# hal0zer0/openwurli

Measured on AMD Instinct MI355X. Metric: audio samples/s, 64-voice full chain (x real-time @48 kHz = value / 48000), higher is better.
Workload: dtype f64

## Files before the change

openwurli_amd/csrc/ow_chain_dev.h:

```cpp
#pragma once
#include "ow_voice_dev.h"

namespace owdev {

OW_DEV double fast_exp(double x0) {
    const double x = clampd(x0, -40.0, 40.0);
    const double SHIFT = 6755399441055744.0;
    const double z = x * 1.4426950408889634 + SHIFT;
    const long long n_i64 = __double_as_longlong(z) - __double_as_longlong(SHIFT);
    const double n = z - SHIFT;
    const double f = (x - n * 0.6931471803691238) - n * 1.9082149292705877e-10;
    const double p = 1.0 + f * (1.0 + f * (0.5 + f * (0.16666666666666607 + f * (0.04166666666665876 + f * 0.008333333333492337))));
    const double pow2n = __longlong_as_double((long long)(((unsigned long long)(1023 + n_i64)) << 52));
    return p * pow2n;
}

__device__ __noinline__ __attribute__((const)) double pnjlim_limited(double vnew, double vold, double vt, double vcrit) {
    if (vold >= 0.0) {
        const double arg = 1.0 + (vnew - vold) / vt;
        return arg > 0.0 ? vold + vt * log(arg) : vcrit;
    }
    return vt * log(vnew / vt);
}
OW_DEV double pnjlim(double vnew, double vold, double vt, double vcrit) {
// ... 383 lines not shown
}
OW_DEV double trem_shunt(double depth, double r_ldr) {
    const double r_upper = 50000.0 * (1.0 - depth);
    const double r_lower = 50000.0 * depth;
    const double top = r_upper > 0.0 ? ow_div(r_upper * 18000.0, r_upper + 18000.0) : 0.0;
    const double branch = 680.0 + r_ldr;
    const double low = r_lower > 0.0 ? ow_div(r_lower * branch, r_lower + branch) : 0.0;
    return top + low;
}

struct Smoother {
    double cur, target, step;
    uint32_t rem;
    OW_DEV double next() {
        if (rem > 0u) {
            cur += step;
            rem -= 1u;
            if (rem == 0u) cur = target;
        }
        return cur;
    }
    OW_DEV void retarget(double t, uint32_t ramp) {
        target = t;
        const double delta = t - cur;
        if (ramp == 0u) { cur = t; rem = 0u; return; }
        step = delta / (double)ramp;
        rem = ramp;
    }
};

OW_DEV double xor32(double x);
OW_DEV double xor32_t(double x) {
#ifdef OW_XOR32_SWAP
    return xor32(x);
#else
    return __shfl_xor(x, 32);
#endif
}
OW_DEV double xor32(double x) {
    const int lo = __double2loint(x), hi = __double2hiint(x);
    const auto a = __builtin_amdgcn_permlane32_swap(lo, lo, false, false);
    const auto b = __builtin_amdgcn_permlane32_swap(hi, hi, false, false);
    const bool low_half = (threadIdx.x & 63) < 32;
    return __hiloint2double(low_half ? b[1] : b[0], low_half ? a[1] : a[0]);
}

#define OW_P_IS 3.03e-14
#define OW_P_VT 0.026
struct DkSt { double j_cin, cin_prev, v[8], i_nl[2], v_nl[2], gm[2]; };
#ifdef OW_DBG_COUNTERS
extern __device__ unsigned long long g_ow_dbg[8];
#endif

OW_DEV double exp_bounded(double x) {
#ifdef OW_LIB_EXP
    return exp(x);
#else
    const double n = rint(x * __longlong_as_double(0x3ff71547652b82feLL));
    double r = __builtin_fma(__longlong_as_double((long long)0xbfe62e42fefa39efULL), n, x);
    r = __builtin_fma(__longlong_as_double((long long)0xbc7abc9e3b39803fULL), n, r);
    double p = __builtin_fma(__longlong_as_double(0x3e5ade156a5dcb37LL), r, __longlong_as_double(0x3e928af3fca7ab0cLL));
    p = __builtin_fma(r, p, __longlong_as_double(0x3ec71dee623fde64LL));
    p = __builtin_fma(r, p, __longlong_as_double(0x3efa01997c89e6b0LL));
    p = __builtin_fma(r, p, __longlong_as_double(0x3f2a01a014761f6eLL));
    p = __builtin_fma(r, p, __longlong_as_double(0x3f56c16c1852b7b0LL));
    p = __builtin_fma(r, p, __longlong_as_double(0x3f81111111122322LL));
    p = __builtin_fma(r, p, __longlong_as_double(0x3fa55555555502a1LL));
    p = __builtin_fma(r, p, __longlong_as_double(0x3fc5555555555511LL));
    p = __builtin_fma(r, p, __longlong_as_double(0x3fe000000000000bLL));
    p = __builtin_fma(r, p, 1.0);
    p = __builtin_fma(r, p, 1.0);
    return ldexp(p, (int)n);
#endif
}
OW_DEV double dk_clamp_vbe(double vbe) { return __builtin_fmin(__builtin_fmax(vbe, -1.0), 0.85); }
OW_DEV double dk_ic(double vbe) {
    return OW_P_IS * (exp_bounded(OW_DIV_C(dk_clamp_vbe(vbe), OW_P_VT)) - 1.0);
}
OW_DEV void dk_ic_gm(double vbe, double& ic, double& gm) {
    const double e = exp_bounded(OW_DIV_C(dk_clamp_vbe(vbe), OW_P_VT));
    ic = OW_P_IS * (e - 1.0);
    gm = (OW_P_IS / OW_P_VT) * e;
}
OW_DEV void dk_refresh_gm(DkSt& st) {
    double ic;
    dk_ic_gm(st.v_nl[0], ic, st.gm[0]);
    dk_ic_gm(st.v_nl[1], ic, st.gm[1]);
}

__device__ inline const OwConsts* k_reload(const OwConsts* K) {
    int z = 0;
    asm volatile("" : "+s"(z));
    return K + z;
}
__device__ inline double dk_step(DkSt& st, double input, double g_ldr, double g_ldr_prev, const OwConsts* __restrict__ K0) {
    const OwConsts* __restrict__ K = k_reload(K0);
    const double (*__restrict__ an)[8] = K->p_a_neg;
    const double* v = st.v;
    double rhs[8];
    rhs[0] = an[0][0] * v[0] + an[0][2] * v[2];
    rhs[1] = an[1][1] * v[1] + an[1][7] * v[7];
    rhs[2] = an[2][0] * v[0] + an[2][2] * v[2] + an[2][5] * v[5];
    rhs[3] = an[3][3] * v[3] + an[3][4] * v[4];
    rhs[4] = an[4][3] * v[3] + an[4][4] * v[4];
    rhs[5] = an[5][2] * v[2] + an[5][5] * v[5] + an[5][6] * v[6];
    rhs[6] = an[6][5] * v[5] + an[6][6] * v[6] + an[6][7] * v[7];
    rhs[7] = an[7][1] * v[1] + an[7][6] * v[6] + an[7][7] * v[7];
    rhs[7] -= g_ldr_prev * st.v[7];
    const double cin_now = K->p_g_cin * input + st.j_cin;
    rhs[0] += cin_now + st.cin_prev;
    rhs[1] += st.i_nl[0];
    rhs[2] -= st.i_nl[0];
    rhs[3] += st.i_nl[1];
    rhs[5] -= st.i_nl[1];
#pragma unroll
    for (int i = 0; i < 8; ++i) rhs[i] += K->p_two_w[i];
    double vpb[8];
    {
        const OwConsts* __restrict__ Kb = k_reload(K0);
#pragma unroll
        for (int i = 0; i < 4; ++i) {
            double sum = 0.0;
#pragma unroll
            for (int j = 0; j < 8; ++j) sum += Kb->p_s[i][j] * rhs[j];
            vpb[i] = sum;
// ... 20 lines not shown
    const double k11 = K->p_k[1][1] - sm_k * K->p_nv_sfb[1] * K->p_sfb_ni[1];
    double vn0 = st.v_nl[0], vn1 = st.v_nl[1];
    double ic0 = st.i_nl[0], ic1 = st.i_nl[1], gm0 = st.gm[0], gm1 = st.gm[1];
    bool done = false;
#ifdef OW_DBG_COUNTERS
    unsigned own_updates = 0u, wave_updates = 0u;
#endif
    for (int iter = 0; iter < 6; ++iter) {
        const double f0 = vn0 - p0 - k00 * ic0 - k01 * ic1;
        const double f1 = vn1 - p1 - k10 * ic0 - k11 * ic1;
        done = done || (fabs(f0) < 1e-9 && fabs(f1) < 1e-9);
        if (__builtin_amdgcn_ballot_w64(!done) == 0ull) break;
#ifdef OW_DBG_COUNTERS
        own_updates += done ? 0u : 1u; wave_updates += 1u;
#endif
        const double j00 = 1.0 - k00 * gm0, j01 = -k01 * gm1, j10 = -k10 * gm0, j11 = 1.0 - k11 * gm1;
        const double det = j00 * j11 - j01 * j10;
        done = done || fabs(det) < 1e-30;
        const double inv_det = ow_div(1.0, det);
        const double n0 = vn0 - inv_det * (j11 * f0 - j01 * f1);
        const double n1 = vn1 - inv_det * (j00 * f1 - j10 * f0);
        vn0 = done ? vn0 : n0;
        vn1 = done ? vn1 : n1;
        dk_ic_gm(vn0, ic0, gm0);
        dk_ic_gm(vn1, ic1, gm1);
    }
#ifdef OW_DBG_COUNTERS
    {
        const int ln = threadIdx.x & 63;
        atomicAdd(&g_ow_dbg[ln < 32 ? 0 : 1], (unsigned long long)own_updates);
        if (ln == 0) { atomicAdd(&g_ow_dbg[2], (unsigned long long)wave_updates); atomicAdd(&g_ow_dbg[3], 1ull); }
        unsigned m = own_updates;
        for (int o = 16; o > 0; o >>= 1) m = max(m, (unsigned)__shfl_xor((int)m, o));
        if (ln == 0) atomicAdd(&g_ow_dbg[4], (unsigned long long)m);
        if (ln == 32) atomicAdd(&g_ow_dbg[5], (unsigned long long)m);
    }
#endif
    K = k_reload(K0);
    const double dot = K->p_sfb_ni[0] * ic0 + K->p_sfb_ni[1] * ic1;
#pragma unroll
    for (int i = 0; i < 8; ++i) {
        const double s_ni_i = ic0 * K->p_sni_d1[i] + ic1 * K->p_sni_d2[i];
        st.v[i] = v_pred[i] + s_ni_i - sm_k * dot * K->p_s_fb_col[i];
    }
    st.cin_prev = cin_now;
    const double dv_cin = input - st.v[0];
    st.j_cin = -K->p_gc_1pc * dv_cin - K->p_c_cin * st.j_cin;
    st.i_nl[0] = ic0; st.i_nl[1] = ic1;
    st.v_nl[0] = vn0; st.v_nl[1] = vn1;
    st.gm[0] = gm0; st.gm[1] = gm1;
    return st.v[6];
}

OW_DEV void dk_rhs(const double (*__restrict__ an)[8], const DkSt& st, double input, double g_ldr_prev, double p_g_cin, double rhs[8], double& cin_now) {
    const double* v = st.v;
    rhs[0] = an[0][0] * v[0] + an[0][2] * v[2];
    rhs[1] = an[1][1] * v[1] + an[1][7] * v[7];
    rhs[2] = an[2][0] * v[0] + an[2][2] * v[2] + an[2][5] * v[5];
    rhs[3] = an[3][3] * v[3] + an[3][4] * v[4];
    rhs[4] = an[4][3] * v[3] + an[4][4] * v[4];
    rhs[5] = an[5][2] * v[2] + an[5][5] * v[5] + an[5][6] * v[6];
    rhs[6] = an[6][5] * v[5] + an[6][6] * v[6] + an[6][7] * v[7];
    rhs[7] = an[7][1] * v[1] + an[7][6] * v[6] + an[7][7] * v[7];
    rhs[7] -= g_ldr_prev * st.v[7];
    cin_now = p_g_cin * input + st.j_cin;
    rhs[0] += cin_now + st.cin_prev;
    rhs[1] += st.i_nl[0];
    rhs[2] -= st.i_nl[0];
    rhs[3] += st.i_nl[1];
    rhs[5] -= st.i_nl[1];
}
OW_DEV void dk_newton_update(double k00, double k01, double k10, double k11, double f0, double f1, bool& done,
                             double& vn0, double& vn1, double& ic0, double& ic1, double& gm0, double& gm1) {
    const double j00 = 1.0 - k00 * gm0, j01 = -k01 * gm1, j10 = -k10 * gm0, j11 = 1.0 - k11 * gm1;
    const double det = j00 * j11 - j01 * j10;
    done = done || fabs(det) < 1e-30;
    const double inv_det = ow_div(1.0, det);
    const double n0 = vn0 - inv_det * (j11 * f0 - j01 * f1);
    const double n1 = vn1 - inv_det * (j00 * f1 - j10 * f0);
    vn0 = done ? vn0 : n0;
    vn1 = done ? vn1 : n1;
    dk_ic_gm(vn0, ic0, gm0);
    dk_ic_gm(vn1, ic1, gm1);
}
OW_DEV double dk_close(const OwConsts* __restrict__ K, DkSt& st, const double v_pred[8], double sm_k, double cin_now, double input,
                       double vn0, double vn1, double ic0, double ic1, double gm0, double gm1) {
    const double dot = K->p_sfb_ni[0] * ic0 + K->p_sfb_ni[1] * ic1;
#pragma unroll
    for (int i = 0; i < 8; ++i) {
        const double s_ni_i = ic0 * K->p_sni_d1[i] + ic1 * K->p_sni_d2[i];
        st.v[i] = v_pred[i] + s_ni_i - sm_k * dot * K->p_s_fb_col[i];
    }
    st.cin_prev = cin_now;
    const double dv_cin = input - st.v[0];
    st.j_cin = -K->p_gc_1pc * dv_cin - K->p_c_cin * st.j_cin;
    st.i_nl[0] = ic0; st.i_nl[1] = ic1;
    st.v_nl[0] = vn0; st.v_nl[1] = vn1;
    st.gm[0] = gm0; st.gm[1] = gm1;
    return st.v[6];
}
__device__ inline void dk_step_pair(DkSt& sa, DkSt& sb, double in_a, double in_b, double g_ldr, double g_ldr_prev,
                                    const OwConsts* __restrict__ K0, double& out_a, double& out_b) {
    const OwConsts* __restrict__ K = k_reload(K0);
    double ra[8], rb[8], cin_a, cin_b;
    dk_rhs(K->p_a_neg, sa, in_a, g_ldr_prev, K->p_g_cin, ra, cin_a);
    dk_rhs(K->p_a_neg, sb, in_b, g_ldr_prev, K->p_g_cin, rb, cin_b);
#pragma unroll
    for (int i = 0; i < 8; ++i) { ra[i] += K->p_two_w[i]; rb[i] += K->p_two_w[i]; }
    double pa[8], pb[8];
    {
        const OwConsts* __restrict__ Kb = k_reload(K0);
#pragma unroll
        for (int i = 0; i < 4; ++i) {
            double sum_a = 0.0, sum_b = 0.0;
#pragma unroll
            for (int j = 0; j < 8; ++j) { const double s = Kb->p_s[i][j]; sum_a += s * ra[j]; sum_b += s * rb[j]; }
            pa[i] = sum_a; pb[i] = sum_b;
        }
        const OwConsts* __restrict__ Kc = k_reload(K0);
#pragma unroll
        for (int i = 4; i < 8; ++i) {
            double sum_a = 0.0, sum_b = 0.0;
#pragma unroll
            for (int j = 0; j < 8; ++j) { const double s = Kc->p_s[i][j]; sum_a += s * ra[j]; sum_b += s * rb[j]; }
            pa[i] = sum_a; pb[i] = sum_b;
        }
    }
    K = k_reload(K0);
    const double sm_k = ow_div(g_ldr, 1.0 + K->p_s_fb_fb * g_ldr);
    const double k00 = K->p_k[0][0] - sm_k * K->p_nv_sfb[0] * K->p_sfb_ni[0];
    const double k01 = K->p_k[0][1] - sm_k * K->p_nv_sfb[0] * K->p_sfb_ni[1];
    const double k10 = K->p_k[1][0] - sm_k * K->p_nv_sfb[1] * K->p_sfb_ni[0];
    const double k11 = K->p_k[1][1] - sm_k * K->p_nv_sfb[1] * K->p_sfb_ni[1];
    const double smv_a = sm_k * pa[7], smv_b = sm_k * pb[7];
#pragma unroll
    for (int i = 0; i < 8; ++i) { const double c = K->p_s_fb_col[i]; pa[i] = pa[i] - smv_a * c; pb[i] = pb[i] - smv_b * c; }
    const double p0a = pa[0] - pa[1], p1a = pa[2] - pa[3];
    const double p0b = pb[0] - pb[1], p1b = pb[2] - pb[3];
    double vn0a = sa.v_nl[0], vn1a = sa.v_nl[1], ic0a = sa.i_nl[0], ic1a = sa.i_nl[1], gm0a = sa.gm[0], gm1a = sa.gm[1];
    double vn0b = sb.v_nl[0], vn1b = sb.v_nl[1], ic0b = sb.i_nl[0], ic1b = sb.i_nl[1], gm0b = sb.gm[0], gm1b = sb.gm[1];
    bool done_a = false, done_b = false;
#pragma unroll
    for (int iter = 0; iter < 6; ++iter) {
        const double f0a = vn0a - p0a - k00 * ic0a - k01 * ic1a;
        const double f1a = vn1a - p1a - k10 * ic0a - k11 * ic1a;
        const double f0b = vn0b - p0b - k00 * ic0b - k01 * ic1b;
        const double f1b = vn1b - p1b - k10 * ic0b - k11 * ic1b;
        done_a = done_a || (fabs(f0a) < 1e-9 && fabs(f1a) < 1e-9);
        done_b = done_b || (fabs(f0b) < 1e-9 && fabs(f1b) < 1e-9);
        if (__builtin_amdgcn_ballot_w64(!(done_a && done_b)) == 0ull) break;
        dk_newton_update(k00, k01, k10, k11, f0a, f1a, done_a, vn0a, vn1a, ic0a, ic1a, gm0a, gm1a);
        dk_newton_update(k00, k01, k10, k11, f0b, f1b, done_b, vn0b, vn1b, ic0b, ic1b, gm0b, gm1b);
    }
    K = k_reload(K0);
    out_a = dk_close(K, sa, pa, sm_k, cin_a, in_a, vn0a, vn1a, ic0a, ic1a, gm0a, gm1a);
    out_b = dk_close(K, sb, pb, sm_k, cin_b, in_b, vn0b, vn1b, ic0b, ic1b, gm0b, gm1b);
}

__device__ __noinline__ void dk_dc_state(const OwConsts* __restrict__ K, double r_ldr, DkSt* out) {
    double w[8][16];
    for (int i = 0; i < 8; ++i)
        for (int j = 0; j < 8; ++j) { w[i][j] = K->p_g_dc_base[i][j]; w[i][8 + j] = (i == j) ? 1.0 : 0.0; }
    w[7][7] += 1.0 / r_ldr;
    for (int col = 0; col < 8; ++col) {
        int piv = col;
        double best = fabs(w[col][col]);
        for (int r = col + 1; r < 8; ++r)
            if (fabs(w[r][col]) > best) { best = fabs(w[r][col]); piv = r; }
        if (piv != col)
            for (int j = 0; j < 16; ++j) { const double t = w[col][j]; w[col][j] = w[piv][j]; w[piv][j] = t; }
        const double d = w[col][col];
        for (int j = 0; j < 16; ++j) w[col][j] /= d;
        for (int r = 0; r < 8; ++r) {
            if (r == col) continue;
            const double f = w[r][col];
            for (int j = 0; j < 16; ++j) w[r][j] -= f * w[col][j];
        }
    }
#define SDC(i, j) w[i][8 + (j)]
    const double kd00 = SDC(0, 1) - SDC(0, 2) - SDC(1, 1) + SDC(1, 2);
    const double kd01 = SDC(0, 3) - SDC(0, 5) - SDC(1, 3) + SDC(1, 5);
    const double kd10 = SDC(2, 1) - SDC(2, 2) - SDC(3, 1) + SDC(3, 2);
    const double kd11 = SDC(2, 3) - SDC(2, 5) - SDC(3, 3) + SDC(3, 5);
    double wv[8], sv[8];
    for (int i = 0; i < 8; ++i) wv[i] = K->p_two_w[i] * 0.5;
    for (int i = 0; i < 8; ++i) {
        double sum = 0.0;
        for (int j = 0; j < 8; ++j) sum += SDC(i, j) * wv[j];
        sv[i] = sum;
    }
    const double pd0 = sv[0] - sv[1], pd1 = sv[2] - sv[3];
    double vn0 = 0.56, vn1 = 0.66;
    for (int iter = 0; iter < 100; ++iter) {
        double ic0, gm0, ic1, gm1;
        dk_ic_gm(vn0, ic0, gm0);
        dk_ic_gm(vn1, ic1, gm1);
        const double f0 = vn0 - pd0 - kd00 * ic0 - kd01 * ic1;
        const double f1 = vn1 - pd1 - kd10 * ic0 - kd11 * ic1;
        if (fabs(f0) < 1e-12 && fabs(f1) < 1e-12) break;
        const double j00 = 1.0 - kd00 * gm0, j01 = -kd01 * gm1, j10 = -kd10 * gm0, j11 = 1.0 - kd11 * gm1;
        const double det = j00 * j11 - j01 * j10;
        const double inv_det = 1.0 / det;
        const double dv0 = inv_det * (j11 * f0 - j01 * f1);
        const double dv1 = inv_det * (j00 * f1 - j10 * f0);
        const double ms = 2.0 * OW_P_VT;
        vn0 -= clampd(dv0, -ms, ms);
        vn1 -= clampd(dv1, -ms, ms);
    }
    const double ic0 = dk_ic(vn0), ic1 = dk_ic(vn1);
    double rhs[8];
    for (int i = 0; i < 8; ++i) rhs[i] = wv[i];
    rhs[1] += ic0; rhs[2] -= ic0; rhs[3] += ic1; rhs[5] -= ic1;
    for (int i = 0; i < 8; ++i) {
        double sum = 0.0;
        for (int j = 0; j < 8; ++j) sum += SDC(i, j) * rhs[j];
        out->v[i] = sum;
    }
#undef SDC
    out->j_cin = K->p_g_cin * out->v[0];
    out->cin_prev = K->p_g_cin * out->v[0];
    out->i_nl[0] = dk_ic(vn0); out->i_nl[1] = dk_ic(vn1);
    out->v_nl[0] = vn0; out->v_nl[1] = vn1;
}
__device__ inline void dk_dc_reset(const OwConsts* __restrict__ K, double r_ldr, DkSt& st) {
    DkSt tmp;
    dk_dc_state(K, r_ldr, &tmp);
    st = tmp;
    dk_refresh_gm(st);
}

OW_DEV double allpass3(const double c0, const double c1, const double c2, double st[3], double x) {
    double y = c0 * x + st[0];
    st[0] = x - c0 * y;
    double y2 = c1 * y + st[1];
    st[1] = y - c1 * y2;
    double y3 = c2 * y2 + st[2];
    st[2] = y2 - c2 * y3;
    return y3;
}
#define OW_OS_A0 0.036681502163648
#define OW_OS_A1 0.248030921580110
#define OW_OS_A2 0.643184620136480
#define OW_OS_B0 0.110377634768680
#define OW_OS_B1 0.420399304190880
#define OW_OS_B2 0.854640112701920


__device__ inline double power_amp(double input) {
    const double A = 19000.0, H = 22.0, TOL = 1e-6;
    const double beta = 220.0 / (220.0 + 15000.0);
    const double clg = A / (1.0 + A * beta);
    double y = clampd(input * clg, -H + TOL, H - TOL);
#ifndef OW_DK_DIVERGENT_NEWTON
    bool done = false;
#endif
    for (int it = 0; it < 8; ++it) {
        const double error = input - beta * y;
        const double v = A * error;
        const double v_sq = v * v;
        const double vt_sq = 0.013 * 0.013;
        const double exp_term = exp(OW_DIV_C(-v_sq, 0.013 * 0.013));
        const double q = 0.1;
        const double cross_gain = q + (1.0 - q) * (1.0 - exp_term);
        const double v_cross = v * cross_gain;
        const double dcross_dv = cross_gain + v * (1.0 - q) * OW_DIV_C(2.0 * v, 0.013 * 0.013) * exp_term;
        const double tanh_val = tanh_fast(OW_DIV_C(v_cross, 22.0));
        const double f_val = H * tanh_val;
        const double f_deriv = (1.0 - tanh_val * tanh_val) * dcross_dv;
        const double residual = y - f_val;
        const double jac = 1.0 + A * beta * f_deriv;
        const double delta = ow_div(residual, jac);
#ifndef OW_DK_DIVERGENT_NEWTON
        y = done ? y : y - delta;
        done = done || fabs(delta) < TOL;
        if (__builtin_amdgcn_ballot_w64(!done) == 0ull) break;
#else
        y -= delta;
        if (fabs(delta) < TOL) break;
#endif
    }
    return OW_DIV_C(y, 22.0);
}

struct Bq { double b0, b1, b2, a1, a2, s1, s2; };
OW_DEV double bq_process(Bq& f, double x) {
    const double y = f.b0 * x + f.s1;
    f.s1 = f.b1 * x - f.a1 * y + f.s2;
    f.s2 = f.b2 * x - f.a2 * y;
    return y;
}
__device__ inline void bq_design(Bq& f, bool highpass, double fc, double q, double sr) {
    const double w0 = 2.0 * 3.14159265358979323846 * fc / sr;
    const double cw = cos(w0), sw = sin(w0);
    const double alpha = sw / (2.0 * q);
    const double a0 = 1.0 + alpha;
    if (highpass) { f.b0 = ((1.0 + cw) / 2.0) / a0; f.b1 = (-(1.0 + cw)) / a0; f.b2 = ((1.0 + cw) / 2.0) / a0; }
    else          { f.b0 = ((1.0 - cw) / 2.0) / a0; f.b1 = (1.0 - cw) / a0;    f.b2 = ((1.0 - cw) / 2.0) / a0; }
    f.a1 = (-2.0 * cw) / a0;
    f.a2 = (1.0 - alpha) / a0;
}
struct SpeakerSt {
    Bq hpf, lpf;
    double character, a2, a3, tc, ts;
};
__device__ inline void speaker_update(SpeakerSt& s, double sr) {
    const double c = s.character;
    bq_design(s.hpf, true, 20.0 * pow(30.0 / 20.0, c), 0.75, sr);
    bq_design(s.lpf, false, 20000.0 * pow(5500.0 / 20000.0, c), 0.707, sr);
    s.a2 = 0.2 * c;
    s.a3 = 0.6 * c;
    s.tc = 2.0 * c;
}
OW_DEV void speaker_set_character(SpeakerSt& s, double ch, double sr) {
    const double c = clampd(ch, 0.0, 1.0);
// ... 23 lines not shown
```

openwurli_amd/csrc/ow_dk_step_debug.h:

```cpp
#pragma once
#include "ow_chain_row.h"

namespace owdev {

enum { DKF_LANE = 0, DKF_PAIR = 1, DKF_WIDE = 2, DKF_ROW = 3 };

template <int FORM>
__global__ __launch_bounds__(64) void k_debug_dk_step(const OwConsts* __restrict__ K, const double* __restrict__ cs_in, const double* __restrict__ input,
                                                      const double* __restrict__ g_ldr, const double* __restrict__ g_ldr_prev, int n,
                                                      double* __restrict__ cs_out, double* __restrict__ out) {
    const int lane = threadIdx.x;
    const long long t = (long long)blockIdx.x * 64 + lane;
    if constexpr (FORM == DKF_LANE) {
        const bool valid = t < n;
        const int c = valid ? (int)t : n - 1;
        DkSt st;
        dk_load(st, cs_in, n, c, 0);
        const double o = dk_step(st, input[c], g_ldr[c], g_ldr_prev[c], K);
        if (valid) { dk_store(st, cs_out, n, c, 0); out[c] = o; }
    } else if constexpr (FORM == DKF_PAIR) {
        const long long ca = 2 * t, cb = 2 * t + 1;
        const bool va = ca < n, vb = cb < n;
        const int a = va ? (int)ca : n - 1, b = vb ? (int)cb : n - 1;
        DkSt sm, ss;
        dk_load(sm, cs_in, n, a, 0);
        dk_load(ss, cs_in, n, b, 0);
        double om, os;
        dk_step_pair(sm, ss, input[a], input[b], g_ldr[a], g_ldr_prev[a], K, om, os);
        if (va) { dk_store(sm, cs_out, n, a, 0); out[a] = om; }
        if (vb) { dk_store(ss, cs_out, n, b, 0); out[b] = os; }
    } else if constexpr (FORM == DKF_WIDE) {
        const int q = lane & 3;
        const long long cw = t >> 2;
        const bool valid = cw < n;
        const int c = valid ? (int)cw : n - 1;
        DkWideRows R;
        dk_wide_rows_load(R, K, q);
        DkSt st;
        dk_load(st, cs_in, n, c, 0);
        const double o = dk_step_wide(st, R, q, input[c], g_ldr[c], g_ldr_prev[c], K);
        if (valid && q == (c & 3)) { dk_store(st, cs_out, n, c, 0); out[c] = o; }
    } else {
        const long long cr = t >> 4;
        const bool valid = cr < n;
        const int c = valid ? (int)cr : n - 1;
        DkRowK R;
        dk_row_consts(R, K, lane);
        DkSt st;
        dk_load(st, cs_in, n, c, 0);
        const double o = dk_step_row(st, R, lane, input[c], g_ldr[c], g_ldr_prev[c]);
        if (valid && (lane & 15) == (c & 15)) { dk_store(st, cs_out, n, c, 0); out[c] = o; }
    }
}

}
```

openwurli_amd/csrc/ow_kernels.h:

```cpp
#pragma once
#include "ow_vm.h"
#include "ow_chain_dev.h"

namespace owdev {

#define OW_DATA_DECL __device__ const
#define OW_GEN_DATA_REINCLUDE
#include "../../data/ow_gen_data.h"
#undef OW_GEN_DATA_REINCLUDE
#undef OW_DATA_DECL

struct OwEngineOut {
    uint64_t silent_mask;
    uint64_t bad_main;
    uint64_t bad_steal;
    uint32_t sum_nonfinite;
    uint32_t out_nonfinite;
    uint32_t transient;
    uint32_t pad;
};

__device__ inline void mlp_raw_scalar(double in0, double in1, double raw[11]) {
    double h1[16], h2[16];
    for (int i = 0; i < 16; ++i) {
// ... 1055 lines not shown
            }
        }
        __syncthreads();
    }
    if (valid) {
        dk_store(st, cs, I, e, role ? CS_P_SHADOW : CS_P_MAIN);
        if (role == 0) {
            for (int i = 0; i < 3; ++i) { CSF(CS_OS_UA + i) = ua[i]; CSF(CS_OS_UB + i) = ub[i]; }
            CSF(CS_P_RLDR) = r_ldr; CSF(CS_P_GLDR) = g_ldr; CSF(CS_P_GPREV) = g_prev;
            smoother_store(sd, cs, I, e, CS_SM_DEPTH);
            const uint64_t fl = dbits(CSF(CS_FLAGS));
            if (fl & 1ull) CSF(CS_FLAGS) = bitsd(fl & ~1ull);
            if (nan_resets) {
                const uint64_t d = dbits(CSF(CS_DIAG));
                CSF(CS_DIAG) = bitsd((d & 0xFFFFFFFFull) | ((uint64_t)((uint32_t)(d >> 32) + nan_resets) << 32));
            }
        }
    }
}

#define OW_PPCHUNK 32
__global__ __launch_bounds__(64) __attribute__((amdgpu_waves_per_eu(2, 2)))
void k_preamp_pair(const OwConsts* __restrict__ K, double* __restrict__ cs, const OwEngineArgs* __restrict__ args,
                   const OwEngineOut* __restrict__ eout, const double* __restrict__ sum, const OwTremSrc tsrc,
                   double* __restrict__ pre, int I, int L, int Lcap, int e0, int ne) {
    __shared__ double tile[64 * (OW_PPCHUNK + 1)];
    const int lane = threadIdx.x;
    const int eb = e0 + blockIdx.x * 64;
    const int e = eb + lane;
    const bool valid = e < e0 + ne;
    const int ec = valid ? e : (e0 + ne - 1);
    const int osr = K->oversample ? 2 : 1;

    DkSt sm, ss;
    double ua[3], ub[3];
    double r_ldr, g_ldr, g_prev;
    Smoother sd;
    {
        const int e = ec;
        smoother_load(sd, cs, I, e, CS_SM_DEPTH);
        if (args[e].set_flags & 1u) sd.retarget(args[e].depth_target, K->ramp_samples);
        dk_load(sm, cs, I, e, CS_P_MAIN);
        dk_load(ss, cs, I, e, CS_P_SHADOW);
        for (int i = 0; i < 3; ++i) { ua[i] = CSF(CS_OS_UA + i); ub[i] = CSF(CS_OS_UB + i); }
        r_ldr = CSF(CS_P_RLDR); g_ldr = CSF(CS_P_GLDR); g_prev = CSF(CS_P_GPREV);
        const uint64_t fl = dbits(CSF(CS_FLAGS));
        if (fl & 1ull) {
            dk_dc_reset(K, r_ldr, sm);
            ss = sm;
            g_ldr = 1.0 / r_ldr; g_prev = g_ldr;
            for (int i = 0; i < 3; ++i) { ua[i] = 0.0; ub[i] = 0.0; }
        }
    }
    uint32_t nan_resets = 0;
    double sh_depth = __longlong_as_double(0x7FF8000000000000LL), sh_top = 0.0, sh_lower = 0.0;
    int rowflag = 0;
    if (valid && !eout[e].sum_nonfinite) rowflag = (args[e].main_mask ? 1 : 0) | (args[e].steal_mask ? 2 : 0);
    const int e_last = e0 + ne - 1;
    const int half = lane >> 5;
    const TremCol tcol = trem_col(tsrc, I, ec);
    double rn[2];
    rn[0] = trem_col_at(tcol, 0u);
    rn[1] = osr == 2 ? trem_col_at(tcol, 1u) : 0.0;
    for (int base = 0; base < L; base += OW_PPCHUNK) {
        const int cn = min(OW_PPCHUNK, L - base);
        const int col = base + min(lane & 31, cn - 1);
#pragma unroll 8
        for (int r = 0; r < 32; ++r) {
            const int row = r + 32 * half;
            const int er = min(eb + row, e_last);
            const int fl_lo = __builtin_amdgcn_readlane(rowflag, r), fl_hi = __builtin_amdgcn_readlane(rowflag, r + 32);
            const int fl = half ? fl_hi : fl_lo;
            const double a = sum[((size_t)0 * I + er) * Lcap + col];
            const double b = sum[((size_t)1 * I + er) * Lcap + col];
            double x = (fl & 1) ? a : 0.0;
            x = (fl & 2) ? x + b : x;
            tile[row * (OW_PPCHUNK + 1) + (lane & 31)] = x;
        }
        __syncthreads();
        for (int n = 0; n < cn; ++n) {
            const double x = tile[lane * (OW_PPCHUNK + 1) + n];
            const double rc[2] = {rn[0], rn[1]};
            {
                const uint32_t nx = (uint32_t)(min(base + n + 1, L - 1) * osr);
                rn[0] = trem_col_at(tcol, nx);
                if (osr == 2) rn[1] = trem_col_at(tcol, nx + 1u);
            }
            const double depth = clampd(sd.next(), 0.0, 1.0);
            if (__builtin_amdgcn_ballot_w64(!(depth == sh_depth)) != 0ull) {
                sh_depth = depth;
                const double r_upper = 50000.0 * (1.0 - depth);
                sh_lower = 50000.0 * depth;
                sh_top = r_upper > 0.0 ? ow_div(r_upper * 18000.0, r_upper + 18000.0) : 0.0;
            }
            double in[2];
            if (osr == 2) {
                in[0] = allpass3(OW_OS_A0, OW_OS_A1, OW_OS_A2, ua, x);
                in[1] = allpass3(OW_OS_B0, OW_OS_B1, OW_OS_B2, ub, x);
            } else {
                in[0] = x;
                in[1] = 0.0;
            }
            for (int j = 0; j < osr; ++j) {
                const size_t idx = (size_t)((base + n) * osr + j);
                const double branch = 680.0 + rc[j];
                const double low = sh_lower > 0.0 ? ow_div(sh_lower * branch, sh_lower + branch) : 0.0;
                const double r_new = fmax(sh_top + low, 1000.0);
                if (fabs(r_new - r_ldr) > 0.01) { r_ldr = r_new; g_ldr = ow_div(1.0, r_new); }
                double om, os;
                dk_step_pair(sm, ss, in[j], 0.0, g_ldr, g_prev, K, om, os);
                g_prev = g_ldr;
                double result = om - os;
                if (!isfinite(result)) {
                    dk_dc_reset(K, r_ldr, sm);
                    ss = sm;
                    g_ldr = 1.0 / r_ldr; g_prev = g_ldr;
                    result = 0.0;
                    nan_resets += 1u;
                }
                if (valid) pre[idx * I + e] = result;
            }
        }
        __syncthreads();
    }
    if (valid) {
        dk_store(sm, cs, I, e, CS_P_MAIN);
        dk_store(ss, cs, I, e, CS_P_SHADOW);
        for (int i = 0; i < 3; ++i) { CSF(CS_OS_UA + i) = ua[i]; CSF(CS_OS_UB + i) = ub[i]; }
        CSF(CS_P_RLDR) = r_ldr; CSF(CS_P_GLDR) = g_ldr; CSF(CS_P_GPREV) = g_prev;
        smoother_store(sd, cs, I, e, CS_SM_DEPTH);
        const uint64_t fl = dbits(CSF(CS_FLAGS));
        if (fl & 1ull) CSF(CS_FLAGS) = bitsd(fl & ~1ull);
        if (nan_resets) {
            const uint64_t d = dbits(CSF(CS_DIAG));
            CSF(CS_DIAG) = bitsd((d & 0xFFFFFFFFull) | ((uint64_t)((uint32_t)(d >> 32) + nan_resets) << 32));
        }
    }
}

#define OW_OCHUNK 64
template <bool SPLIT, bool PAIR = false>
__global__ __launch_bounds__(64) void k_post(const OwConsts* __restrict__ K, double* __restrict__ cs, const OwEngineArgs* __restrict__ args,
                                             OwEngineOut* __restrict__ eout, const double* __restrict__ pre, float* __restrict__ out, int I, int L,
                                             int Lcap, int e0, int ne, float* __restrict__ out2 = nullptr, size_t ld2 = 0) {
    constexpr int NROWS = SPLIT ? 32 : 64;
    __shared__ float tile[NROWS * (OW_OCHUNK + 1)];
    const int lane = threadIdx.x;
    const int el = SPLIT ? (lane & 31) : lane;
    const int phase = SPLIT ? (lane >> 5) : 0;
    const int eb = e0 + blockIdx.x * NROWS;
    const int e_raw = eb + el;
    const bool valid = e_raw < e0 + ne;
    const int e = valid ? e_raw : (e0 + ne - 1);
    static_assert(!(SPLIT && PAIR), "PAIR is the lane = engine form of the oversampled chain");
    const int osr = (SPLIT || PAIR) ? 2 : 1;
    const double sr = K->sr;
    const double thermal_alpha = K->spk_thermal_alpha;

    double da[3], db[3], dd;
    for (int i = 0; i < 3; ++i) { da[i] = CSF(CS_OS_DA + i); db[i] = CSF(CS_OS_DB + i); }
    dd = CSF(CS_OS_DD);
    SpeakerSt sp;
    {
// ... 80 lines not shown
```

openwurli_amd/csrc/ow_voice_dev.h:

```cpp
#pragma once
#include <hip/hip_runtime.h>
#include "ow_types.h"

namespace owdev {

#define OW_DEV __device__ __forceinline__
#define OW_HD __host__ __device__ __forceinline__
#define OW_HDI __host__ __device__ inline

OW_DEV double ow_div(double a, double b) {
#ifdef OW_IEEE_DIV
    return a / b;
#else
    double y = __builtin_amdgcn_rcp(b);
    double e = __builtin_fma(-b, y, 1.0);
    y = __builtin_fma(y, e, y);
    e = __builtin_fma(-b, y, 1.0);
    y = __builtin_fma(y, e, y);
    const double q = a * y;
    const double r = __builtin_fma(-b, q, a);
    return __builtin_amdgcn_div_fixup(__builtin_fma(r, y, q), b, a);
#endif
}
OW_DEV double ow_rcp_refined(double b) {
// ... 387 lines not shown
    const double hfsq = 0.5 * f * f;
    const double dk = (double)k;
    return dk * 6.93147180369123816490e-01 - ((hfsq - (s * (hfsq + R) + dk * 1.90821492927058770002e-10)) - f);
}
OW_DEV double exp_nonpos(double x) {
    const double n = rint(x * __longlong_as_double(0x3ff71547652b82feLL));
    double r = __builtin_fma(__longlong_as_double((long long)0xbfe62e42fefa39efULL), n, x);
    r = __builtin_fma(__longlong_as_double((long long)0xbc7abc9e3b39803fULL), n, r);
    double p = __builtin_fma(__longlong_as_double(0x3e5ade156a5dcb37LL), r, __longlong_as_double(0x3e928af3fca7ab0cLL));
    p = fma_k(r, p, __longlong_as_double(0x3ec71dee623fde64LL));
    p = fma_k(r, p, __longlong_as_double(0x3efa01997c89e6b0LL));
    p = fma_k(r, p, __longlong_as_double(0x3f2a01a014761f6eLL));
    p = fma_k(r, p, __longlong_as_double(0x3f56c16c1852b7b0LL));
    p = fma_k(r, p, __longlong_as_double(0x3f81111111122322LL));
    p = fma_k(r, p, __longlong_as_double(0x3fa55555555502a1LL));
    p = fma_k(r, p, __longlong_as_double(0x3fc5555555555511LL));
    p = fma_k(r, p, __longlong_as_double(0x3fe000000000000bLL));
    p = __builtin_fma(r, p, 1.0);
    p = __builtin_fma(r, p, 1.0);
    return ldexp(p, (int)n);
}
__device__ __noinline__ __attribute__((const)) double onset_gain(double n, double onset_inc, double onset_exp) {
#ifdef OW_LIB_POW
    const double cosine = 0.5 * (1.0 - cos(n * onset_inc));
    if (onset_exp <= 1.001) return cosine;
    if (onset_exp >= 1.999) return cosine * cosine;
    return pow(cosine, onset_exp);
#else
    const double cosine = 0.5 * (1.0 - cos_0_pi(n * onset_inc));
    if (onset_exp <= 1.001) return cosine;
    if (onset_exp >= 1.999) return cosine * cosine;
    if (!(cosine > 0.0)) return 0.0;
    return exp_nonpos(onset_exp * log_unit(cosine));
#endif
}
__device__ __noinline__ __attribute__((const)) double exp_neg(double x) { return exp(-x); }
OW_DEV double exp_neg_poly(double x) {
    const double y = -x;
    double p = __builtin_fma(y, 2.50521083854417187751e-08, 2.75573192239858906526e-07);
    p = __builtin_fma(y, p, 2.75573192239858906526e-06);
    p = __builtin_fma(y, p, 2.48015873015873015873e-05);
    p = __builtin_fma(y, p, 1.98412698412698412698e-04);
    p = __builtin_fma(y, p, 1.38888888888888888889e-03);
    p = __builtin_fma(y, p, 8.33333333333333333333e-03);
    p = __builtin_fma(y, p, 4.16666666666666666667e-02);
    p = __builtin_fma(y, p, 1.66666666666666666667e-01);
    p = __builtin_fma(y, p, 0.5);
    p = __builtin_fma(y, p, 1.0);
    return __builtin_fma(y, p, 1.0);
}
OW_DEV double exp_neg_small(double x) { return __builtin_expect(!(x <= 0.125), 0) ? exp_neg(x) : exp_neg_poly(x); }
OW_DEV double damper_ramp_pos(double t, double ramp) { return ow_div(t, ramp); }
__device__ __noinline__ __attribute__((const)) double noise_fade_env(double t) { return 0.5 * (1.0 - cos(3.14159265358979323846 * t)); }
OW_DEV double tanh_fast(double x) {
#ifdef OW_LIB_TANH
    return tanh(x);
#else
    double ax = fabs(x);
    ax = ax > 20.0 ? 20.0 : ax;
    const double y = ax + ax;
    const double n = rint(y * __longlong_as_double(0x3ff71547652b82feLL));
    double r = __builtin_fma(__longlong_as_double((long long)0xbfe62e42fefa39efULL), n, y);
    r = __builtin_fma(__longlong_as_double((long long)0xbc7abc9e3b39803fULL), n, r);
    double q = 1.0 / 6227020800.0;
    q = __builtin_fma(q, r, 1.0 / 479001600.0);
    q = __builtin_fma(q, r, 1.0 / 39916800.0);
    q = __builtin_fma(q, r, 1.0 / 3628800.0);
    q = __builtin_fma(q, r, 1.0 / 362880.0);
    q = __builtin_fma(q, r, 1.0 / 40320.0);
    q = __builtin_fma(q, r, 1.0 / 5040.0);
    q = __builtin_fma(q, r, 1.0 / 720.0);
    q = __builtin_fma(q, r, 1.0 / 120.0);
    q = __builtin_fma(q, r, 1.0 / 24.0);
    q = __builtin_fma(q, r, 1.0 / 6.0);
    q = __builtin_fma(q, r, 0.5);
    const double em1 = __builtin_fma(r * r, q, r);
    const double s = __longlong_as_double((long long)(1023 + (int)n) << 52);
    const double z = __builtin_fma(s, em1, s - 1.0);
    const double d = z + 2.0;
    const double d_lo = z <= 2.0 ? z - (d - 2.0) : 0.0;
    double rc = __builtin_amdgcn_rcp(d);
    double e = __builtin_fma(-d, rc, 1.0);
    rc = __builtin_fma(rc, e, rc);
    e = __builtin_fma(-d, rc, 1.0);
    rc = __builtin_fma(rc, e, rc);
    const double q0 = z * rc;
    double res = __builtin_fma(-d, q0, z);
    res = __builtin_fma(-d_lo, q0, res);
    const double t = __builtin_fma(res, rc, q0);
    return copysign(t, x);
#endif
}
__device__ __noinline__ __attribute__((const)) double pickup_saturate_hi(double y) {
    const double ay = fabs(y);
    const double range = 0.98 - 0.94;
    return copysign(0.94 + range * tanh_fast(OW_DIV_C(ay - 0.94, 0.98 - 0.94)), y);
}

#define OW_LCOEF_ROWS 19
OW_DEV void lcoef_load(double* __restrict__ lcoef, const double* __restrict__ rec) {
    for (int i = 0; i < 5; ++i) lcoef[i * 64] = rec[(VF_NB0 + i) * 64];
    for (int i = 0; i < 7; ++i) { lcoef[(5 + i) * 64] = rec[(VF_DRATE + i) * 64]; lcoef[(12 + i) * 64] = rec[(VF_DMULT + i) * 64]; }
}

struct VoiceRegs {
    double s[7], c[7], env[7], drift[7], cos_inc[7], sin_inc[7], phase_inc[7], amp[7], decay[7];
    double ci[7], si[7];
    double onset_inc, onset_exp, dramp, dcount, q, ds, gain;
    double namp, ns1, ns2;
    double beta, jrev, jdiff, ndecay;
    uint64_t sample, onset_n;
    uint32_t jitter_state, noise_rng, noise_rem, noise_fade, flags, midi;

    OW_DEV void load(const double* __restrict__ rec) {
#pragma unroll
        for (int i = 0; i < 7; ++i) {
            s[i] = rec[(VF_S + i) * 64]; c[i] = rec[(VF_C + i) * 64]; env[i] = rec[(VF_ENV + i) * 64];
            drift[i] = rec[(VF_DRIFT + i) * 64]; cos_inc[i] = rec[(VF_COS_INC + i) * 64]; sin_inc[i] = rec[(VF_SIN_INC + i) * 64];
            phase_inc[i] = rec[(VF_PHASE_INC + i) * 64]; amp[i] = rec[(VF_AMP + i) * 64]; decay[i] = rec[(VF_DECAY + i) * 64];
        }
        onset_inc = rec[VF_ONSET_INC * 64]; onset_exp = rec[VF_ONSET_EXP * 64];
        dramp = rec[VF_DRAMP * 64]; dcount = rec[VF_DCOUNT * 64];
        q = rec[VF_Q * 64]; ds = rec[VF_DS * 64]; gain = rec[VF_GAIN * 64];
        beta = rec[VF_BETA * 64]; jrev = rec[VF_JREV * 64]; jdiff = rec[VF_JDIFF * 64]; ndecay = rec[VF_NDECAY * 64];
        namp = rec[VF_NAMP * 64];
        ns1 = rec[VF_NS1 * 64]; ns2 = rec[VF_NS2 * 64];
        sample = dbits(rec[VF_SAMPLE * 64]); onset_n = dbits(rec[VF_ONSET_N * 64]);
        const uint64_t r = dbits(rec[VF_RNG * 64]); jitter_state = (uint32_t)r; noise_rng = (uint32_t)(r >> 32);
// ... 145 lines not shown
```

Baseline: 3.753 billion.

## Hand-schedule scalar constant loads in DK step and inline exp polynomials

Hoists the sparse A-matrix entries, two_w, s_fb_col and g_cin into per-thread VGPR-pinned registers, loaded once per kernel instead of on every DK pair step. It streams the S-matrix rows and the Newton constants through double-buffered s_load_dwordx16 inline asm, with explicit waitcnt so scalar fetches overlap the vector FMAs. It also replaces a library exp with an inline polynomial exp_any, and forces FMA chains in tanh and exp to be emitted as explicit v_fma_f64 asm. The intent is to cut scalar-cache load latency and register pressure from repeated K reloads, at the cost of more held VGPRs and fragile hand-written asm that depends on the OwConsts layout.

```diff
diff --git a/openwurli_amd/csrc/ow_chain_dev.h b/openwurli_amd/csrc/ow_chain_dev.h
--- a/openwurli_amd/csrc/ow_chain_dev.h
+++ b/openwurli_amd/csrc/ow_chain_dev.h
@@ -459,25 +459,42 @@
 extern __device__ unsigned long long g_ow_dbg[8];
 #endif
 
+template <bool F3>
+OW_DEV double exp_core(double x) {
+    const double n = rint(x * __longlong_as_double(0x3ff71547652b82feLL));
+    double r = __builtin_fma(__longlong_as_double((long long)0xbfe62e42fefa39efULL), n, x);
+    r = __builtin_fma(__longlong_as_double((long long)0xbc7abc9e3b39803fULL), n, r);
+#define OW_EXP_STEP(c) p = F3 ? fma3(r, p, __longlong_as_double(c)) : __builtin_fma(r, p, __longlong_as_double(c))
+    const double c11 = __longlong_as_double(0x3e5ade156a5dcb37LL), c10 = __longlong_as_double(0x3e928af3fca7ab0cLL);
+    double p = F3 ? fma3(c11, r, c10) : __builtin_fma(c11, r, c10);
+    OW_EXP_STEP(0x3ec71dee623fde64LL);
+    OW_EXP_STEP(0x3efa01997c89e6b0LL);
+    OW_EXP_STEP(0x3f2a01a014761f6eLL);
+    OW_EXP_STEP(0x3f56c16c1852b7b0LL);
+    OW_EXP_STEP(0x3f81111111122322LL);
+    OW_EXP_STEP(0x3fa55555555502a1LL);
+    OW_EXP_STEP(0x3fc5555555555511LL);
+    OW_EXP_STEP(0x3fe000000000000bLL);
+#undef OW_EXP_STEP
+    p = __builtin_fma(r, p, 1.0);
+    p = __builtin_fma(r, p, 1.0);
+    return ldexp(p, (int)n);
+}
 OW_DEV double exp_bounded(double x) {
 #ifdef OW_LIB_EXP
     return exp(x);
 #else
-    const double n = rint(x * __longlong_as_double(0x3ff71547652b82feLL));
-    double r = __builtin_fma(__longlong_as_double((long long)0xbfe62e42fefa39efULL), n, x);
-    r = __builtin_fma(__longlong_as_double((long long)0xbc7abc9e3b39803fULL), n, r);
-    double p = __builtin_fma(__longlong_as_double(0x3e5ade156a5dcb37LL), r, __longlong_as_double(0x3e928af3fca7ab0cLL));
-    p = __builtin_fma(r, p, __longlong_as_double(0x3ec71dee623fde64LL));
-    p = __builtin_fma(r, p, __longlong_as_double(0x3efa01997c89e6b0LL));
-    p = __builtin_fma(r, p, __longlong_as_double(0x3f2a01a014761f6eLL));
-    p = __builtin_fma(r, p, __longlong_as_double(0x3f56c16c1852b7b0LL));
-    p = __builtin_fma(r, p, __longlong_as_double(0x3f81111111122322LL));
-    p = __builtin_fma(r, p, __longlong_as_double(0x3fa55555555502a1LL));
-    p = __builtin_fma(r, p, __longlong_as_double(0x3fc5555555555511LL));
-    p = __builtin_fma(r, p, __longlong_as_double(0x3fe000000000000bLL));
-    p = __builtin_fma(r, p, 1.0);
-    p = __builtin_fma(r, p, 1.0);
-    return ldexp(p, (int)n);
+    return exp_core<false>(x);
+#endif
+}
+OW_DEV double exp_any(double x) {
+#ifdef OW_LIB_EXP
+    return exp(x);
+#else
+    double z = exp_core<true>(x);
+    z = x > 1024.0 ? __longlong_as_double(0x7ff0000000000000LL) : z;
+    z = x < -1075.0 ? 0.0 : z;
+    return z;
 #endif
 }
 OW_DEV double dk_clamp_vbe(double vbe) { return __builtin_fmin(__builtin_fmax(vbe, -1.0), 0.85); }
@@ -604,16 +621,44 @@
     return st.v[6];
 }
 
-OW_DEV void dk_rhs(const double (*__restrict__ an)[8], const DkSt& st, double input, double g_ldr_prev, double p_g_cin, double rhs[8], double& cin_now) {
+struct DkPairRes { double an[20], two_w[8], s_fb_col[8], g_cin; };
+__device__ inline void dk_pair_res_load(DkPairRes& R, const OwConsts* __restrict__ K) {
+    const double (*__restrict__ an)[8] = K->p_a_neg;
+    const double a[20] = {an[0][0], an[0][2], an[1][1], an[1][7], an[2][0], an[2][2], an[2][5], an[3][3], an[3][4], an[4][3],
+                          an[4][4], an[5][2], an[5][5], an[5][6], an[6][5], an[6][6], an[6][7], an[7][1], an[7][6], an[7][7]};
+#pragma unroll
+    for (int i = 0; i < 20; ++i) { double x = a[i]; asm volatile("" : "+v"(x)); R.an[i] = x; }
+#pragma unroll
+    for (int i = 0; i < 8; ++i) {
+        double w = K->p_two_w[i], c = K->p_s_fb_col[i];
+        asm volatile("" : "+v"(w));
+        asm volatile("" : "+v"(c));
+        R.two_w[i] = w; R.s_fb_col[i] = c;
+    }
+    double g = K->p_g_cin;
+    asm volatile("" : "+v"(g));
+    R.g_cin = g;
+}
+typedef double ow_sd8 __attribute__((ext_vector_type(8)));
+typedef double ow_sd4 __attribute__((ext_vector_type(4)));
+typedef double ow_sd2 __attribute__((ext_vector_type(2)));
+#define OW_KOFF(field) ((int)__builtin_offsetof(OwConsts, field))
+#define OW_SWAIT_FETCH8D(nxt, off, cur, xa, xb) \
+    asm volatile("s_waitcnt lgkmcnt(0)\n\ts_load_dwordx16 %0, %4, %5" : "=&s"(nxt), "+s"(cur), "+v"(xa), "+v"(xb) : "s"(K0), "i"(off))
+#define OW_S_ROW(i, row) { double sum_a = 0.0, sum_b = 0.0; \
+    _Pragma("unroll") for (int j = 0; j < 8; ++j) { const double s = row[j]; sum_a += s * ra[j]; sum_b += s * rb[j]; } \
+    pa[i] = sum_a; pb[i] = sum_b; }
+
+OW_DEV void dk_rhs(const double* __restrict__ an, const DkSt& st, double input, double g_ldr_prev, double p_g_cin, double rhs[8], double& cin_now) {
     const double* v = st.v;
-    rhs[0] = an[0][0] * v[0] + an[0][2] * v[2];
-    rhs[1] = an[1][1] * v[1] + an[1][7] * v[7];
-    rhs[2] = an[2][0] * v[0] + an[2][2] * v[2] + an[2][5] * v[5];
-    rhs[3] = an[3][3] * v[3] + an[3][4] * v[4];
-    rhs[4] = an[4][3] * v[3] + an[4][4] * v[4];
-    rhs[5] = an[5][2] * v[2] + an[5][5] * v[5] + an[5][6] * v[6];
-    rhs[6] = an[6][5] * v[5] + an[6][6] * v[6] + an[6][7] * v[7];
-    rhs[7] = an[7][1] * v[1] + an[7][6] * v[6] + an[7][7] * v[7];
+    rhs[0] = an[0] * v[0] + an[1] * v[2];
+    rhs[1] = an[2] * v[1] + an[3] * v[7];
+    rhs[2] = an[4] * v[0] + an[5] * v[2] + an[6] * v[5];
+    rhs[3] = an[7] * v[3] + an[8] * v[4];
+    rhs[4] = an[9] * v[3] + an[10] * v[4];
+    rhs[5] = an[11] * v[2] + an[12] * v[5] + an[13] * v[6];
+    rhs[6] = an[14] * v[5] + an[15] * v[6] + an[16] * v[7];
+    rhs[7] = an[17] * v[1] + an[18] * v[6] + an[19] * v[7];
     rhs[7] -= g_ldr_prev * st.v[7];
     cin_now = p_g_cin * input + st.j_cin;
     rhs[0] += cin_now + st.cin_prev;
@@ -635,60 +680,74 @@
     dk_ic_gm(vn0, ic0, gm0);
     dk_ic_gm(vn1, ic1, gm1);
 }
-OW_DEV double dk_close(const OwConsts* __restrict__ K, DkSt& st, const double v_pred[8], double sm_k, double cin_now, double input,
+OW_DEV double dk_close(const double sfb_ni[2], const ow_sd8& sni_d1, const ow_sd8& sni_d2, double p_gc_1pc, double p_c_cin,
+                       const double* __restrict__ s_fb_col, DkSt& st, const double v_pred[8], double sm_k, double cin_now, double input,
                        double vn0, double vn1, double ic0, double ic1, double gm0, double gm1) {
-    const double dot = K->p_sfb_ni[0] * ic0 + K->p_sfb_ni[1] * ic1;
+    const double dot = sfb_ni[0] * ic0 + sfb_ni[1] * ic1;
 #pragma unroll
     for (int i = 0; i < 8; ++i) {
-        const double s_ni_i = ic0 * K->p_sni_d1[i] + ic1 * K->p_sni_d2[i];
-        st.v[i] = v_pred[i] + s_ni_i - sm_k * dot * K->p_s_fb_col[i];
+        const double s_ni_i = ic0 * sni_d1[i] + ic1 * sni_d2[i];
+        st.v[i] = v_pred[i] + s_ni_i - sm_k * dot * s_fb_col[i];
     }
     st.cin_prev = cin_now;
     const double dv_cin = input - st.v[0];
-    st.j_cin = -K->p_gc_1pc * dv_cin - K->p_c_cin * st.j_cin;
+    st.j_cin = -p_gc_1pc * dv_cin - p_c_cin * st.j_cin;
     st.i_nl[0] = ic0; st.i_nl[1] = ic1;
     st.v_nl[0] = vn0; st.v_nl[1] = vn1;
     st.gm[0] = gm0; st.gm[1] = gm1;
     return st.v[6];
 }
 __device__ inline void dk_step_pair(DkSt& sa, DkSt& sb, double in_a, double in_b, double g_ldr, double g_ldr_prev,
-                                    const OwConsts* __restrict__ K0, double& out_a, double& out_b) {
-    const OwConsts* __restrict__ K = k_reload(K0);
+                                    const OwConsts* __restrict__ K0, const DkPairRes& R, double& out_a, double& out_b) {
+    ow_sd8 s0, s1;
+    asm volatile("s_load_dwordx16 %0, %9, %10"
+                 : "=s"(s0), "+v"(sa.v[0]), "+v"(sa.v[1]), "+v"(sa.v[3]), "+v"(sa.v[5]), "+v"(sb.v[0]), "+v"(sb.v[1]), "+v"(sb.v[3]), "+v"(sb.v[5])
+                 : "s"(K0), "i"(OW_KOFF(p_s)));
     double ra[8], rb[8], cin_a, cin_b;
-    dk_rhs(K->p_a_neg, sa, in_a, g_ldr_prev, K->p_g_cin, ra, cin_a);
-    dk_rhs(K->p_a_neg, sb, in_b, g_ldr_prev, K->p_g_cin, rb, cin_b);
-#pragma unroll
-    for (int i = 0; i < 8; ++i) { ra[i] += K->p_two_w[i]; rb[i] += K->p_two_w[i]; }
+    dk_rhs(R.an, sa, in_a, g_ldr_prev, R.g_cin, ra, cin_a);
+    dk_rhs(R.an, sb, in_b, g_ldr_prev, R.g_cin, rb, cin_b);
+#pragma unroll
+    for (int i = 0; i < 8; ++i) { ra[i] += R.two_w[i]; rb[i] += R.two_w[i]; }
     double pa[8], pb[8];
-    {
-        const OwConsts* __restrict__ Kb = k_reload(K0);
-#pragma unroll
-        for (int i = 0; i < 4; ++i) {
-            double sum_a = 0.0, sum_b = 0.0;
-#pragma unroll
-            for (int j = 0; j < 8; ++j) { const double s = Kb->p_s[i][j]; sum_a += s * ra[j]; sum_b += s * rb[j]; }
-            pa[i] = sum_a; pb[i] = sum_b;
-        }
-        const OwConsts* __restrict__ Kc = k_reload(K0);
-#pragma unroll
-        for (int i = 4; i < 8; ++i) {
-            double sum_a = 0.0, sum_b = 0.0;
-#pragma unroll
-            for (int j = 0; j < 8; ++j) { const double s = Kc->p_s[i][j]; sum_a += s * ra[j]; sum_b += s * rb[j]; }
-            pa[i] = sum_a; pb[i] = sum_b;
-        }
-    }
-    K = k_reload(K0);
-    const double sm_k = ow_div(g_ldr, 1.0 + K->p_s_fb_fb * g_ldr);
-    const double k00 = K->p_k[0][0] - sm_k * K->p_nv_sfb[0] * K->p_sfb_ni[0];
-    const double k01 = K->p_k[0][1] - sm_k * K->p_nv_sfb[0] * K->p_sfb_ni[1];
-    const double k10 = K->p_k[1][0] - sm_k * K->p_nv_sfb[1] * K->p_sfb_ni[0];
-    const double k11 = K->p_k[1][1] - sm_k * K->p_nv_sfb[1] * K->p_sfb_ni[1];
+    OW_SWAIT_FETCH8D(s1, OW_KOFF(p_s) + 1 * 64, s0, ra[7], rb[7]);
+    OW_S_ROW(0, s0)
+    OW_SWAIT_FETCH8D(s0, OW_KOFF(p_s) + 2 * 64, s1, pa[0], pb[0]);
+    OW_S_ROW(1, s1)
+    OW_SWAIT_FETCH8D(s1, OW_KOFF(p_s) + 3 * 64, s0, pa[1], pb[1]);
+    OW_S_ROW(2, s0)
+    OW_SWAIT_FETCH8D(s0, OW_KOFF(p_s) + 4 * 64, s1, pa[2], pb[2]);
+    OW_S_ROW(3, s1)
+    OW_SWAIT_FETCH8D(s1, OW_KOFF(p_s) + 5 * 64, s0, pa[3], pb[3]);
+    OW_S_ROW(4, s0)
+    OW_SWAIT_FETCH8D(s0, OW_KOFF(p_s) + 6 * 64, s1, pa[4], pb[4]);
+    OW_S_ROW(5, s1)
+    OW_SWAIT_FETCH8D(s1, OW_KOFF(p_s) + 7 * 64, s0, pa[5], pb[5]);
+    OW_S_ROW(6, s0)
+    ow_sd4 kk, kf;
+    ow_sd2 kn;
+    static_assert(OW_KOFF(p_nv_sfb) == OW_KOFF(p_s_fb_fb) + 8 && OW_KOFF(p_sfb_ni) == OW_KOFF(p_s_fb_fb) + 24, "OwConsts layout");
+    asm volatile("s_waitcnt lgkmcnt(0)\n\ts_load_dwordx8 %0, %6, %7\n\ts_load_dwordx8 %1, %6, %8\n\ts_load_dwordx4 %2, %6, %9"
+                 : "=&s"(kk), "=&s"(kf), "=&s"(kn), "+s"(s1), "+v"(pa[6]), "+v"(pb[6])
+                 : "s"(K0), "i"(OW_KOFF(p_k)), "i"(OW_KOFF(p_s_fb_fb)), "i"(OW_KOFF(p_s_fb_fb) + 32));
+    OW_S_ROW(7, s1)
+    ow_sd8 d1, d2;
+    ow_sd2 cc;
+    static_assert(OW_KOFF(p_gc_1pc) == OW_KOFF(p_c_cin) + 8, "OwConsts layout");
+    asm volatile("s_waitcnt lgkmcnt(0)\n\ts_load_dwordx16 %0, %8, %9\n\ts_load_dwordx16 %1, %8, %10\n\ts_load_dwordx4 %2, %8, %11"
+                 : "=&s"(d1), "=&s"(d2), "=&s"(cc), "+s"(kk), "+s"(kf), "+s"(kn), "+v"(pa[7]), "+v"(pb[7])
+                 : "s"(K0), "i"(OW_KOFF(p_sni_d1)), "i"(OW_KOFF(p_sni_d2)), "i"(OW_KOFF(p_c_cin)));
+    const double p_s_fb_fb = kf[0], p_nv_sfb0 = kf[1], p_nv_sfb1 = kf[2], p_sfb_ni0 = kf[3], p_sfb_ni1 = kn[0];
+    const double sm_k = ow_div(g_ldr, 1.0 + p_s_fb_fb * g_ldr);
+    double k00 = kk[0] - sm_k * p_nv_sfb0 * p_sfb_ni0;
+    double k01 = kk[1] - sm_k * p_nv_sfb0 * p_sfb_ni1;
+    double k10 = kk[2] - sm_k * p_nv_sfb1 * p_sfb_ni0;
+    double k11 = kk[3] - sm_k * p_nv_sfb1 * p_sfb_ni1;
     const double smv_a = sm_k * pa[7], smv_b = sm_k * pb[7];
 #pragma unroll
-    for (int i = 0; i < 8; ++i) { const double c = K->p_s_fb_col[i]; pa[i] = pa[i] - smv_a * c; pb[i] = pb[i] - smv_b * c; }
-    const double p0a = pa[0] - pa[1], p1a = pa[2] - pa[3];
-    const double p0b = pb[0] - pb[1], p1b = pb[2] - pb[3];
+    for (int i = 0; i < 8; ++i) { const double c = R.s_fb_col[i]; pa[i] = pa[i] - smv_a * c; pb[i] = pb[i] - smv_b * c; }
+    double p0a = pa[0] - pa[1], p1a = pa[2] - pa[3];
+    double p0b = pb[0] - pb[1], p1b = pb[2] - pb[3];
+    asm volatile("s_waitcnt lgkmcnt(0)" : "+s"(d1), "+s"(d2), "+s"(cc), "+v"(k11), "+v"(p1a), "+v"(p1b), "+v"(pa[7]), "+v"(pb[7]));
     double vn0a = sa.v_nl[0], vn1a = sa.v_nl[1], ic0a = sa.i_nl[0], ic1a = sa.i_nl[1], gm0a = sa.gm[0], gm1a = sa.gm[1];
     double vn0b = sb.v_nl[0], vn1b = sb.v_nl[1], ic0b = sb.i_nl[0], ic1b = sb.i_nl[1], gm0b = sb.gm[0], gm1b = sb.gm[1];
     bool done_a = false, done_b = false;
@@ -704,10 +763,12 @@
         dk_newton_update(k00, k01, k10, k11, f0a, f1a, done_a, vn0a, vn1a, ic0a, ic1a, gm0a, gm1a);
         dk_newton_update(k00, k01, k10, k11, f0b, f1b, done_b, vn0b, vn1b, ic0b, ic1b, gm0b, gm1b);
     }
-    K = k_reload(K0);
-    out_a = dk_close(K, sa, pa, sm_k, cin_a, in_a, vn0a, vn1a, ic0a, ic1a, gm0a, gm1a);
-    out_b = dk_close(K, sb, pb, sm_k, cin_b, in_b, vn0b, vn1b, ic0b, ic1b, gm0b, gm1b);
-}
+    const double sfb_ni[2] = {p_sfb_ni0, p_sfb_ni1};
+    out_a = dk_close(sfb_ni, d1, d2, cc[1], cc[0], R.s_fb_col, sa, pa, sm_k, cin_a, in_a, vn0a, vn1a, ic0a, ic1a, gm0a, gm1a);
+    out_b = dk_close(sfb_ni, d1, d2, cc[1], cc[0], R.s_fb_col, sb, pb, sm_k, cin_b, in_b, vn0b, vn1b, ic0b, ic1b, gm0b, gm1b);
+}
+#undef OW_S_ROW
+#undef OW_SWAIT_FETCH8D
 
 __device__ __noinline__ void dk_dc_state(const OwConsts* __restrict__ K, double r_ldr, DkSt* out) {
     double w[8][16];
@@ -811,7 +872,7 @@
         const double v = A * error;
         const double v_sq = v * v;
         const double vt_sq = 0.013 * 0.013;
-        const double exp_term = exp(OW_DIV_C(-v_sq, 0.013 * 0.013));
+        const double exp_term = exp_any(OW_DIV_C(-v_sq, 0.013 * 0.013));
         const double q = 0.1;
         const double cross_gain = q + (1.0 - q) * (1.0 - exp_term);
         const double v_cross = v * cross_gain;
diff --git a/openwurli_amd/csrc/ow_dk_step_debug.h b/openwurli_amd/csrc/ow_dk_step_debug.h
--- a/openwurli_amd/csrc/ow_dk_step_debug.h
+++ b/openwurli_amd/csrc/ow_dk_step_debug.h
@@ -25,8 +25,10 @@
         DkSt sm, ss;
         dk_load(sm, cs_in, n, a, 0);
         dk_load(ss, cs_in, n, b, 0);
+        DkPairRes R;
+        dk_pair_res_load(R, K);
         double om, os;
-        dk_step_pair(sm, ss, input[a], input[b], g_ldr[a], g_ldr_prev[a], K, om, os);
+        dk_step_pair(sm, ss, input[a], input[b], g_ldr[a], g_ldr_prev[a], K, R, om, os);
         if (va) { dk_store(sm, cs_out, n, a, 0); out[a] = om; }
         if (vb) { dk_store(ss, cs_out, n, b, 0); out[b] = os; }
     } else if constexpr (FORM == DKF_WIDE) {
diff --git a/openwurli_amd/csrc/ow_kernels.h b/openwurli_amd/csrc/ow_kernels.h
--- a/openwurli_amd/csrc/ow_kernels.h
+++ b/openwurli_amd/csrc/ow_kernels.h
@@ -1131,6 +1131,8 @@
             for (int i = 0; i < 3; ++i) { ua[i] = 0.0; ub[i] = 0.0; }
         }
     }
+    DkPairRes R;
+    dk_pair_res_load(R, K);
     uint32_t nan_resets = 0;
     double sh_depth = __longlong_as_double(0x7FF8000000000000LL), sh_top = 0.0, sh_lower = 0.0;
     int rowflag = 0;
@@ -1182,12 +1184,12 @@
             }
             for (int j = 0; j < osr; ++j) {
                 const size_t idx = (size_t)((base + n) * osr + j);
-                const double branch = 680.0 + rc[j];
+                const double branch = 680.0 + (j ? rc[1] : rc[0]);
                 const double low = sh_lower > 0.0 ? ow_div(sh_lower * branch, sh_lower + branch) : 0.0;
                 const double r_new = fmax(sh_top + low, 1000.0);
                 if (fabs(r_new - r_ldr) > 0.01) { r_ldr = r_new; g_ldr = ow_div(1.0, r_new); }
                 double om, os;
-                dk_step_pair(sm, ss, in[j], 0.0, g_ldr, g_prev, K, om, os);
+                dk_step_pair(sm, ss, j ? in[1] : in[0], 0.0, g_ldr, g_prev, K, R, om, os);
                 g_prev = g_ldr;
                 double result = om - os;
                 if (!isfinite(result)) {
diff --git a/openwurli_amd/csrc/ow_voice_dev.h b/openwurli_amd/csrc/ow_voice_dev.h
--- a/openwurli_amd/csrc/ow_voice_dev.h
+++ b/openwurli_amd/csrc/ow_voice_dev.h
@@ -463,6 +463,18 @@
 OW_DEV double exp_neg_small(double x) { return __builtin_expect(!(x <= 0.125), 0) ? exp_neg(x) : exp_neg_poly(x); }
 OW_DEV double damper_ramp_pos(double t, double ramp) { return ow_div(t, ramp); }
 __device__ __noinline__ __attribute__((const)) double noise_fade_env(double t) { return 0.5 * (1.0 - cos(3.14159265358979323846 * t)); }
+#ifndef OW_FMA3
+#define OW_FMA3 1
+#endif
+OW_DEV double fma3(double a, double b, double c) {
+#if OW_FMA3
+    double d;
+    [[clang::noconvergent]] { asm("v_fma_f64 %0, %1, %2, %3" : "=v"(d) : "v"(a), "v"(b), "v"(c)); }
+    return d;
+#else
+    return __builtin_fma(a, b, c);
+#endif
+}
 OW_DEV double tanh_fast(double x) {
 #ifdef OW_LIB_TANH
     return tanh(x);
@@ -474,17 +486,17 @@
     double r = __builtin_fma(__longlong_as_double((long long)0xbfe62e42fefa39efULL), n, y);
     r = __builtin_fma(__longlong_as_double((long long)0xbc7abc9e3b39803fULL), n, r);
     double q = 1.0 / 6227020800.0;
-    q = __builtin_fma(q, r, 1.0 / 479001600.0);
-    q = __builtin_fma(q, r, 1.0 / 39916800.0);
-    q = __builtin_fma(q, r, 1.0 / 3628800.0);
-    q = __builtin_fma(q, r, 1.0 / 362880.0);
-    q = __builtin_fma(q, r, 1.0 / 40320.0);
-    q = __builtin_fma(q, r, 1.0 / 5040.0);
-    q = __builtin_fma(q, r, 1.0 / 720.0);
-    q = __builtin_fma(q, r, 1.0 / 120.0);
-    q = __builtin_fma(q, r, 1.0 / 24.0);
-    q = __builtin_fma(q, r, 1.0 / 6.0);
-    q = __builtin_fma(q, r, 0.5);
+    q = fma3(q, r, 1.0 / 479001600.0);
+    q = fma3(q, r, 1.0 / 39916800.0);
+    q = fma3(q, r, 1.0 / 3628800.0);
+    q = fma3(q, r, 1.0 / 362880.0);
+    q = fma3(q, r, 1.0 / 40320.0);
+    q = fma3(q, r, 1.0 / 5040.0);
+    q = fma3(q, r, 1.0 / 720.0);
+    q = fma3(q, r, 1.0 / 120.0);
+    q = fma3(q, r, 1.0 / 24.0);
+    q = fma3(q, r, 1.0 / 6.0);
+    q = fma3(q, r, 0.5);
     const double em1 = __builtin_fma(r * r, q, r);
     const double s = __longlong_as_double((long long)(1023 + (int)n) << 52);
     const double z = __builtin_fma(s, em1, s - 1.0);
```

New measurement: 3.857 billion (median of 6 runs). 2.8% higher.
